# NinV/Background-Debiased-Video-CIL

Hardware: AMD Instinct MI355X
Metric: clips/sec fwd+bwd TSM-R50 8x224^2 bs32/GPU (higher is better)
Workload: dtype f32; 1 GPU; TSM-ResNet50 fwd+bwd+SGD step, synthetic 32x8x3x224x224 clips per GPU, 101 classes, SimpleLinear+CrossEntropyLoss, dropout 0.5, random-init weights; fp32 tensors, accumulators and results; conv products: fp32 via 3xbf16 split, 6 MFMA products, fp32 accumulate (dropped terms <= 2^-24 relative); conv_arith=bf16x3, clips_per_gpu=32, global_batch=32, parallelism=dp1

## Files before the change

### background-debiased-video-cil_amd/_lib.py

```python
from __future__ import annotations

import ctypes
import os
from ctypes import POINTER, Structure, c_char, c_char_p, c_float, c_int, c_int32, c_int64, c_size_t, c_uint16, c_uint64, c_void_p

_HERE = os.path.dirname(os.path.abspath(__file__))
_OVERRIDE = os.environ.get('BDVCIL_LIB_PATH')
LIB_PATH = _OVERRIDE or os.path.join(_HERE, 'csrc', 'libbdvcil_hip.so')
ABI_VERSION = 33

_lib = None


class ConvGeom(Structure):
    _fields_ = [(n, c_int32) for n in
                ('N', 'H', 'W', 'Cin', 'Ho', 'Wo', 'Cout', 'R', 'S', 'stride', 'pad', 'T', 'fold', 'pad_w', 'Rt', 'st_t', 'act_dtype')]

    def key(self):
        return tuple(getattr(self, n) for n, _ in self._fields_)


class ConvPlan(Structure):
    _fields_ = [(n, c_int32) for n in ('family', 'reads_planes', 'stat_rows', 'splits', 'pre_ok')] + [('kernel', c_char * 128)]


P = c_void_p
_F3 = c_float * 3


class ConvAffine(Structure):
    _fields_ = [('scale', c_void_p), ('shift', c_void_p), ('residual', c_void_p), ('relu', c_int32)]


class BnStatFuse(Structure):
    _fields_ = [('y', c_void_p), ('relu_mask', c_void_p), ('mean', c_void_p), ('invstd', c_void_p), ('partial', c_void_p),
                ('relu_scale', c_void_p), ('relu_shift', c_void_p)]

class JpegInfo(Structure):
    _fields_ = [('width', c_int32), ('height', c_int32), ('ncomp', c_int32), ('h', c_int32 * 3), ('v', c_int32 * 3),
                ('blocks_w', c_int32 * 3), ('blocks_h', c_int32 * 3), ('down_w', c_int32 * 3), ('down_h', c_int32 * 3),
                ('qt', (c_uint16 * 64) * 3), ('coef_offset', c_int64 * 3), ('coef_count', c_int64)]

    def geometry_key(self):
        return (self.width, self.height, self.ncomp, tuple(self.h), tuple(self.v))


SIGNATURES = {
    'bdv_last_error': (c_char_p, []),
    'bdv_abi_version': (c_int, []),
    'bdv_source_hash': (c_char_p, []),
    'bdv_conv_workspace_bytes': (c_size_t, [POINTER(ConvGeom), c_int]),
    'bdv_conv_plan_query': (c_int, [POINTER(ConvGeom), c_int, c_int, c_int, POINTER(ConvPlan)]),
    'bdv_conv_fprop': (c_int, [P, P, P, POINTER(ConvGeom), P, POINTER(ConvAffine), P, c_size_t, P]),
    'bdv_conv_dgrad': (c_int, [P, P, P, P, P, POINTER(ConvGeom), POINTER(BnStatFuse), P, c_size_t, P]),
    'bdv_conv_weight_planes_bytes': (c_size_t, [POINTER(ConvGeom)]),
    'bdv_conv_split_weights': (c_int, [P, POINTER(ConvGeom), P, P, P]),
    'bdv_conv_debug_force_tile': (c_int, [c_int]),
    'bdv_conv_fprop_pl': (c_int, [P, P, P, P, POINTER(ConvGeom), P, POINTER(ConvAffine), P, c_size_t, c_int, P, P, P]),
    'bdv_conv_dgrad_pl': (c_int, [P, P, P, P, P, P, POINTER(ConvGeom), POINTER(BnStatFuse), P, c_size_t, c_int, P]),
    'bdv_conv_wgrad': (c_int, [P, P, P, c_float, POINTER(ConvGeom), P, c_size_t, P]),
    'bdv_conv_wgrad_partial': (c_int, [P, P, POINTER(ConvGeom), P, c_size_t, P]),
    'bdv_conv_wgrad_partial_pl': (c_int, [P, P, POINTER(ConvGeom), P, c_size_t, c_int, P, P, P]),
    'bdv_wgrad_reduce_batched': (c_int, [P, P, P, P, c_int, c_float, P]),
    'bdv_f16x2_amax': (c_int, [P, c_int64, P, P]),
    'bdv_f16x2_scale': (c_float, [c_float]),
    'bdv_conv_split_weights_f16x2': (c_int, [P, POINTER(ConvGeom), P, P, P]),
    'bdv_conv_fprop_f16x2': (c_int, [P, P, P, P, P, POINTER(ConvGeom), P, POINTER(ConvAffine), P, c_size_t, P, P, P]),
    'bdv_conv_dgrad_f16x2': (c_int, [P, P, P, P, P, P, P, POINTER(ConvGeom), POINTER(BnStatFuse), P, c_size_t, P]),
    'bdv_conv_wgrad_partial_f16x2': (c_int, [P, P, P, P, POINTER(ConvGeom), P, c_size_t, P, P, P]),
    'bdv_bn_workspace_bytes': (c_size_t, [c_int64, c_int]),
    'bdv_bn_train_stats': (c_int, [P, c_int64, c_int, P, P, c_float, c_float, P, P, P, P, P, P, P, c_size_t, P]),
    'bdv_bn_train_finalize': (c_int, [P, c_int, c_int64, c_int, P, P, c_float, c_float, P, P, P, P, P, P, P]),
    'bdv_bn_eval_params': (c_int, [c_int, P, P, P, P, c_float, P, P, P]),
    'bdv_bn_apply': (c_int, [P, P, P, P, P, P, P, P, c_int64, c_int, c_int, c_int, P]),
    'bdv_bn_backward': (c_int, [P, P, P, P, P, P, P, P, P, c_float, c_int64, c_int, c_int, P, c_int, P, P, P, c_size_t, c_int, P]),
    'bdv_bn_finalize_scratch_bytes': (c_size_t, [c_int]),
    'bdv_bn_finalize_splits': (c_int, [c_int, c_int]),
    'bdv_bn_train_finalize_split': (c_int, [P, c_int, c_int64, c_int, P, P, c_float, c_float, P, P, P, P, P, P, c_int, P, c_size_t, P]),
    'bdv_bn_backward_split': (c_int, [P, P, P, P, P, P, P, P, P, c_float, c_int64, c_int, c_int, P, c_int, P, P, P, c_size_t, c_int,
                                      c_int, P, c_size_t, P]),
    'bdv_bn_pair_workspace_bytes': (c_size_t, [c_int64, c_int]),
    'bdv_bn_backward_pair': (c_int, [P, P, P, P, P, P, P, c_int, P, P, P, P, P, P, P, P, P, P, c_int64, c_int, P, c_size_t, c_int, c_int,
                                     P, c_size_t, P]),
    'bdv_bn_eval_backward': (c_int, [P, P, P, P, P, P, P, P, P, P, P, c_float, c_int64, c_int, P, c_size_t, c_int, c_int, P, c_size_t, P]),
    'bdv_bn_backward_maxpool_split': (c_int, [P, P, P, P, P, P, P, P, P, P, c_float, c_int, c_int, c_int, c_int, P, c_size_t, c_int,
                                              c_int, P, c_size_t, P]),
    'bdv_bn_backward_maxpool': (c_int, [P, P, P, P, P, P, P, P, P, P, c_float, c_int, c_int, c_int, c_int, P, c_size_t, c_int, P]),
    'bdv_relu_bwd': (c_int, [P, P, P, P, c_int64, c_int, P]),
    'bdv_add': (c_int, [P, P, P, c_int64, c_int, P]),
    'bdv_nchw3_to_nhwc4': (c_int, [P, P, c_int, c_int, c_int, P]),
# ... 37 lines not shown
    'bdv_lsc_loss': (c_int, [P, P, P, c_float, c_int, P, P, P, P, c_int, c_int, P]),
    'bdv_softce_loss': (c_int, [P, P, P, P, P, c_int, c_int, P]),
    'bdv_icarl_targets': (c_int, [P, P, c_int, P, P, c_int, c_int, P]),
    'bdv_acm_targets': (c_int, [P, P, P, c_float, P, c_int, c_int, P]),
    'bdv_softmax_mean': (c_int, [P, P, c_int, c_int, c_int, c_int, P]),
    'bdv_topk_acc': (c_int, [P, P, P, c_int, c_int, P]),
    'bdv_repr_from_features': (c_int, [P, P, P, c_int, c_int, c_int, c_int, P]),
    'bdv_nme_workspace_bytes': (c_size_t, [c_int, c_int]),
    'bdv_nme_classify': (c_int, [P, P, P, P, c_int, c_int, c_int, c_int, P, c_size_t, P]),
    'bdv_class_means': (c_int, [P, P, P, c_int, c_int, c_int, P]),
    'bdv_herding_workspace_bytes': (c_size_t, [c_int, c_int]),
    'bdv_herding_select': (c_int, [P, c_int, c_int, c_int, c_int, P, P, P, P, c_size_t, P]),
    'bdv_randaug_workspace_bytes': (c_size_t, [c_int, c_int, c_int, c_int]),
    'bdv_randaug_apply': (c_int, [P, P, P, P, c_int, c_int, c_int, c_int, P, c_size_t, P]),
    'bdv_reduce_workspace_bytes': (c_size_t, []),
    'bdv_kd_mse_fwd': (c_int, [P, P, P, c_int64, P, c_size_t, c_int, P]),
    'bdv_kd_mse_bwd': (c_int, [P, P, P, c_float, P, c_int64, c_int, P]),
    'bdv_multi_sqnorm': (c_int, [P, P, c_int, P, P, c_size_t, P]),
    'bdv_clip_coef': (c_int, [P, c_float, c_float, P, P]),
    'bdv_multi_sgd': (c_int, [P, P, P, P, P, P, c_int, c_float, c_float, P, P]),
    'bdv_gradcam_map': (c_int, [P, P, P, c_int, c_int, c_int, P]),
    'bdv_gradcam_minmax': (c_int, [P, c_int, c_int, c_int, c_int, c_int, c_int, P, P]),
    'bdv_gradcam_workspace_bytes': (c_size_t, [c_int, c_int, c_int]),
    'bdv_gradcam_render': (c_int, [P, P, c_int, c_int, c_int, c_int, c_int, c_int, P, P, P, c_float, _F3, _F3, P, P, P, P, P, c_int, P, P,
                                   c_size_t, P]),
}


class HipExtensionError(RuntimeError):
    pass


HASHED_SOURCES = ('conv_mfma.hip', 'bn.hip', 'pool_frontend.hip', 'head_loss.hip', 'repr.hip', 'augment.hip', 'optim.hip', 'jpeg.hip',
                  'background.hip', 'actor_cut_mix.hip', 'sim_cam.hip', 'ragged.hip', 'gradcam.hip', 'api_common.cpp', 'common.h', 'resize_linear.h', 'Makefile', '../../include/bdvcil_hip.h')


def source_hash():
    import hashlib
    h = hashlib.sha256()
    base = os.path.join(_HERE, 'csrc')
    for name in HASHED_SOURCES:
        path = os.path.join(base, name)
        if not os.path.exists(path):
            return None
        with open(path, 'rb') as f:
            h.update(f.read())
    return h.hexdigest()


def lib():
    global _lib
    if _lib is None:
        if not os.path.exists(LIB_PATH):
            raise HipExtensionError(
                f'HIP extension not built: {LIB_PATH} is missing. Run `python -c "import __graft_entry__ as g; '
                f'g.build()"` (or `make -C {os.path.dirname(LIB_PATH)}`). There is no CPU fallback.')
        handle = ctypes.CDLL(LIB_PATH)
        for name, (res, args) in SIGNATURES.items():
            fn = getattr(handle, name)
            fn.restype = res
            fn.argtypes = args
        if handle.bdv_abi_version() != ABI_VERSION:
            raise HipExtensionError(f'ABI mismatch: library {handle.bdv_abi_version()} != binding {ABI_VERSION}')
        want, have = source_hash(), handle.bdv_source_hash().decode()
        if want is not None and want != have and not _OVERRIDE:
            raise HipExtensionError(f'stale library: {LIB_PATH} was built from other sources (hash {have[:12]}, in-tree '
                                    f'{want[:12]}). Rebuild: make -C {os.path.dirname(LIB_PATH)}')
# ... 9 lines not shown
```

### background-debiased-video-cil_amd/csrc/conv_mfma.hip

```cpp
#include <stdlib.h>
#include <string.h>
#include "common.h"

#ifdef BDV_STAMPS
__device__ unsigned long long* g_stamp_buf = nullptr;
__device__ int g_stamp_cap = 0;
#define BDV_STAMP(slot)                                                                                                          \
  do {                                                                                                                           \
    if (threadIdx.x == 0 && g_stamp_buf != nullptr && (int)(blockIdx.x + gridDim.x * blockIdx.y) < g_stamp_cap) {                 \
      unsigned long long* q_ = g_stamp_buf + (size_t)(blockIdx.x + gridDim.x * blockIdx.y) * 8;                                  \
      if ((slot) == 4) asm volatile("s_waitcnt vmcnt(0)" ::: "memory");                                                          \
      q_[slot] = __builtin_amdgcn_s_memtime();                                                                                   \
      if ((slot) == 0) { q_[5] = __builtin_amdgcn_s_memrealtime(); q_[7] = __builtin_amdgcn_s_getreg((4 << 0) | (0 << 6) | (31 << 11)); } \
      if ((slot) == 4) q_[6] = __builtin_amdgcn_s_memrealtime();                                                                 \
    }                                                                                                                            \
  } while (0)
#else
#define BDV_STAMP(slot) do { } while (0)
#endif

namespace {

constexpr int BK = 32;

struct Geom {
  int N, H, W, Cin, Ho, Wo, Cout, R, S, stride, pad, pad_w, T, fold;
  int Rt, st_t;
  float rcp_RS, rcp_S;
  int M;
  int Ktot;
  float rcp_HoWo, rcp_Wo;
  int stagger;
};

typedef unsigned int u32x4 __attribute__((ext_vector_type(4)));
constexpr int kOOB = (int)0x80000000;

__device__ __forceinline__ float4 buf_load16(__amdgpu_buffer_rsrc_t rsrc, int voff, int soff) {
  const u32x4 v = __builtin_amdgcn_raw_buffer_load_b128(rsrc, voff, soff, 0);
  return make_float4(__uint_as_float(v.x), __uint_as_float(v.y), __uint_as_float(v.z), __uint_as_float(v.w));
}

__device__ __forceinline__ void buf_store16(__amdgpu_buffer_rsrc_t rsrc, int voff, float4 v) {
  u32x4 d;
  d.x = __float_as_uint(v.x);
  d.y = __float_as_uint(v.y);
  d.z = __float_as_uint(v.z);
  d.w = __float_as_uint(v.w);
  __builtin_amdgcn_raw_buffer_store_b128(d, rsrc, voff, 0, 0);
}

typedef unsigned int u32x2v __attribute__((ext_vector_type(2)));
template <int ES>
__device__ __forceinline__ float4 buf_ld4(__amdgpu_buffer_rsrc_t rsrc, int voff) {
  if constexpr (ES == 4) {
    return buf_load16(rsrc, voff, 0);
  } else {
    const u32x2v v = __builtin_amdgcn_raw_buffer_load_b64(rsrc, voff, 0, 0);
    return bdv_widen_bf16x4(v.x, v.y);
  }
}
template <int ES>
__device__ __forceinline__ void buf_st4(__amdgpu_buffer_rsrc_t rsrc, int voff, float4 v) {
  if constexpr (ES == 4) {
    buf_store16(rsrc, voff, v);
// ... 1663 lines not shown
      __syncthreads();
      store(0, PlSet0{});
      load(PlSet0{});
      mma(1);
      __syncthreads();
    }
  } else {
    for (; i + 4 < n; i += 2) {
      mma(0);
      store(1, PlSet1{});
      load(PlSet1{});
      __syncthreads();
      mma(1);
      store(0, PlSet0{});
      load(PlSet0{});
      __syncthreads();
    }
  }
  for (; i < n; i += 2) {
    mma(0);
    if (i + 1 < n) store(1, PlSet1{});
    if (i + 3 < n) load(PlSet1{});
    __syncthreads();
    if (i + 1 >= n) break;
    mma(1);
    if (i + 2 < n) store(0, PlSet0{});
    if (i + 4 < n) load(PlSet0{});
    __syncthreads();
  }
}

constexpr int pl_waves_per_simd(int waves, int np, bool fits128) { return np == 1 && waves == 8 && fits128 ? 4 : waves == 4 ? 2 : waves / 4; }

template <int BM, int BN, int WM, int WN, int NBUF, int NP = 3, bool PRE = false, int ES = 4, typename PT = Bf16Pieces>
__global__ __launch_bounds__(64 * WM * WN, pl_waves_per_simd(WM * WN, NP, BN == 64 || (BM == 128 && BN == 256))) void conv_fprop_pl_kernel(const void* __restrict__ x,
                                                                                      const unsigned short* __restrict__ wp,
                                                                                      void* __restrict__ y, Geom g, int NT, Work wk,
                                                                                      float* __restrict__ slab, FpropEpi epi,
                                                                                      PieceScales ps) {
  static_assert(!kF16<PT> || (NP == 2 && !PRE && ES == 4), "fp16 pieces: two per operand, fp32 tensors, no BatchNorm in the loader");
  constexpr int NTHR = 64 * WM * WN;
  constexpr int TM = BM / WM / 32, TN = BN / WN / 32;
  constexpr int KG = ES == 2 ? 4 : 8;
  constexpr int AP = BM * KG / NTHR;
  constexpr int BPP = (BN * 4 + NTHR - 1) / NTHR;
  constexpr int PA = BM * 64, PB = BN * 64, STAGE = NP * (PA + PB);
  constexpr int SMEM = NBUF * STAGE >= WM * 32 * BN * 4 ? NBUF * STAGE : WM * 32 * BN * 4;
  static_assert(AP >= 1 && SMEM <= 160 * 1024, "tile / epilogue staging do not fit");
  __shared__ __attribute__((aligned(16))) unsigned char smem_b[SMEM];
  float* const smem = reinterpret_cast<float*>(smem_b);

  BDV_STAMP(0);
  const int nk = g.Ktot / BK;
  const WorkItem it = get_work(blockIdx.x, wk, nk);
  const int mt = it.tile / NT, nt = it.tile - mt * NT;

  const int tid = threadIdx.x;
  const int lane = tid & 63, wave = tid >> 6;
  const int wm = wave / WN, wn = wave % WN;
  const int arow = tid / KG, kg = tid % KG;
  const int brow = tid >> 2, bc = tid & 3;
  const int HoWo = g.Ho * g.Wo;
  static_assert(ES == 4 || (NP == 1 && !PRE), "bf16 storage: single-product arithmetic only");
  const int frame_bytes = g.H * g.W * g.Cin * ES;
  const int plane_bytes = g.Cout * g.Ktot * 2;

  const __amdgpu_buffer_rsrc_t xr = __builtin_amdgcn_make_buffer_rsrc((void*)x, 0, g.N * frame_bytes, 0x00020000);
  const __amdgpu_buffer_rsrc_t wr = __builtin_amdgcn_make_buffer_rsrc((void*)wp, 0, 3 * plane_bytes, 0x00020000);

  int a_base[AP], a_t[AP], a_hi0[AP], a_wi0[AP];
#pragma unroll
  for (int p = 0; p < AP; ++p) {
    const int m = mt * BM + arow + (NTHR / KG) * p;
    const bool ok = m < g.M;
    int n, rem, ho, wo;
    fast_divmod(ok ? m : 0, HoWo, g.rcp_HoWo, n, rem);
    fast_divmod(rem, g.Wo, g.rcp_Wo, ho, wo);
    a_t[p] = n % g.T;
    a_hi0[p] = ok ? ho * g.stride - g.pad : -(1 << 20);
    a_wi0[p] = wo * g.stride - g.pad_w;
// ... 48 lines not shown
    chunk += wr_;
  };
  const int st_a = ES == 2 ? pl_off(arow, kg) : pl_off(arow, kg >> 1) + 8 * (kg & 1), st_b = pl_off(brow, bc);
  const int fa[2] = {pl_frag_off(32 * wm, 0, lane), pl_frag_off(32 * wm, 1, lane)};
  const int fb[2] = {pl_frag_off(32 * wn, 0, lane), pl_frag_off(32 * wn, 1, lane)};
  const float sc_a = f16x2_scale<PT>(ps.a);
  auto store = [&](int stage, auto set) __attribute__((always_inline)) {
    constexpr int SET = decltype(set)::value;
    unsigned char* const As = smem_b + stage * STAGE;
    unsigned char* const Bs = As + NP * PA;
#pragma unroll
    for (int p = 0; p < AP; ++p) {
      float4 v = ra[SET][p];
      if constexpr (PRE) {
        const bool ok = (pvalid[SET] >> p) & 1u;
        v.x = ok ? fmaxf(fmaf(v.x, psc[SET].x, psh[SET].x), 0.f) : 0.f;
        v.y = ok ? fmaxf(fmaf(v.y, psc[SET].y, psh[SET].y), 0.f) : 0.f;
        v.z = ok ? fmaxf(fmaf(v.z, psc[SET].z, psh[SET].z), 0.f) : 0.f;
        v.w = ok ? fmaxf(fmaf(v.w, psc[SET].w, psh[SET].w), 0.f) : 0.f;
      }
      if constexpr (ES == 2) *reinterpret_cast<float4*>(As + st_a + (NTHR / KG) * p * 64) = v;
      else pl_split_store_at<NP, PT>(As + st_a + (NTHR / KG) * p * 64, PA, v, sc_a);
    }
    if (b_active) {
#pragma unroll
      for (int pl = 0; pl < NP; ++pl)
#pragma unroll
        for (int q = 0; q < BPP; ++q) *reinterpret_cast<u32x4*>(Bs + st_b + (pl * PB + (NTHR / 4) * q * 64)) = rb[SET][pl * BPP + q];
    }
  };
  f32x16 acc[TM][TN];
  zero_acc<TM, TN>(acc);

  if constexpr (NBUF == 2) {
    pl_pipeline2(it.ke - it.kb, load, store, [&](int stage) __attribute__((always_inline)) {
      mma_stage_pl<BM, BN, WM, WN, NP, PT>(smem_b + stage * STAGE, smem_b + stage * STAGE + NP * PA, acc, fa, fb);
    }, g.stagger != 0 && wave >= WM * WN / 2);
  } else {
    load(PlSet0{});
    for (int kt = it.kb; kt < it.ke; ++kt) {
      __syncthreads();
      store(0, PlSet0{});
      __syncthreads();
      if (kt == it.kb) BDV_STAMP(1);
      if (kt + 1 < it.ke) load(PlSet0{});
      mma_stage_pl<BM, BN, WM, WN, NP, PT>(smem_b, smem_b + NP * PA, acc, fa, fb);
    }
  }
  BDV_STAMP(2);
  f16x2_unscale<PT>(acc, ps);

  if (it.pslot >= 0) {
    store_partial<TM, TN, NTHR>(slab, it.pslot, acc, tid);
    return;
  }
  fprop_epilogue<BM, BN, WM, WN, ES>(acc, smem, y, g, epi, mt, nt, tid);
  BDV_STAMP(3);
  BDV_STAMP(4);
}

template <int BM, int BN, int WM, int WN, int NBUF, int NP = 3, int ES = 4, typename PT = Bf16Pieces>
__global__ __launch_bounds__(64 * WM * WN, BM == 64 ? 4 : pl_waves_per_simd(WM * WN, NP, BN == 64)) void conv_dgrad_pl_kernel(const void* __restrict__ dy,
                                                                                      const unsigned short* __restrict__ dp,
                                                                                      void* __restrict__ dx,
                                                                                      const void* __restrict__ add_src,
                                                                                      const uint32_t* __restrict__ add_mask, Geom g,
                                                                                      int NT, Work wk, float* __restrict__ slab,
                                                                                      BnStat stat, PieceScales ps) {
  static_assert(!kF16<PT> || (NP == 2 && ES == 4), "fp16 pieces: two per operand, fp32 tensors");
  constexpr int NTHR = 64 * WM * WN;
  constexpr int TM = BM / WM / 32, TN = BN / WN / 32;
  constexpr int KG = ES == 2 ? 4 : 8;
  constexpr int AP = BM * KG / NTHR;
  constexpr int BPP = (BN * 4 + NTHR - 1) / NTHR;
  constexpr int PA = BM * 64, PB = BN * 64, STAGE = NP * (PA + PB);
  constexpr int SMEM = NBUF * STAGE >= WM * 32 * BN * 4 ? NBUF * STAGE : WM * 32 * BN * 4;
  static_assert(AP >= 1 && SMEM <= 160 * 1024, "tile / epilogue staging do not fit");
  __shared__ __attribute__((aligned(16))) unsigned char smem_b[SMEM];
  float* const smem = reinterpret_cast<float*>(smem_b);

  BDV_STAMP(0);
  const int st = g.stride;
  const int ph = blockIdx.y / st, pw = blockIdx.y - ph * st;
  const int Hc = (g.H - ph + st - 1) / st, Wc = (g.W - pw + st - 1) / st;
  const int Mc = g.N * Hc * Wc;
  const int MT = (Mc + BM - 1) / BM;
  const int r0 = (ph + g.pad) % st, s0 = (pw + g.pad_w) % st;
  const int nr = r0 < g.R ? (g.R - r0 + st - 1) / st : 0;
  const int ns = s0 < g.S ? (g.S - s0 + st - 1) / st : 0;
  const int bh = (ph + g.pad - r0) / st, bw = (pw + g.pad_w - s0) / st;
  const int ntap = nr * ns;
  const int nk = ntap * g.Cout / BK;

  int mt, nt;
  WorkItem it;
  if (st == 1) {
    it = get_work(blockIdx.x, wk, nk);
    mt = it.tile / NT;
    nt = it.tile - mt * NT;
  } else {
    const int id = blockIdx.x;
    const int xcd = id & 7, jj = id >> 3;
    mt = (jj / NT) * 8 + xcd;
    nt = jj % NT;
    if (mt >= MT) return;
    it.tile = 0;
    it.kb = 0;
    it.ke = nk;
    it.pslot = -1;
// ... 55 lines not shown
      for (int q = 0; q < BPP; ++q) rb[SET][pl * BPP + q] = __builtin_amdgcn_raw_buffer_load_b128(wr, b_base[q] + pl * plane_bytes, koff_b, 0);
    is += 1;
    const int w1 = (is == ns) ? 1 : 0;
    is = w1 ? 0 : is;
    ir += w1;
    const int w2 = (ir == nr) ? 1 : 0;
    ir = w2 ? 0 : ir;
    chunk += w2;
  };
  const int st_a = ES == 2 ? pl_off(arow, kg) : pl_off(arow, kg >> 1) + 8 * (kg & 1), st_b = pl_off(brow, bc);
  const int fa[2] = {pl_frag_off(32 * wm, 0, lane), pl_frag_off(32 * wm, 1, lane)};
  const int fb[2] = {pl_frag_off(32 * wn, 0, lane), pl_frag_off(32 * wn, 1, lane)};
  const float sc_a = f16x2_scale<PT>(ps.a);
  auto store = [&](int stage, auto set) __attribute__((always_inline)) {
    constexpr int SET = decltype(set)::value;
    unsigned char* const As = smem_b + stage * STAGE;
    unsigned char* const Bs = As + NP * PA;
#pragma unroll
    for (int p = 0; p < AP; ++p) {
      if constexpr (ES == 2) *reinterpret_cast<float4*>(As + st_a + (NTHR / KG) * p * 64) = ra[SET][p];
      else pl_split_store_at<NP, PT>(As + st_a + (NTHR / KG) * p * 64, PA, ra[SET][p], sc_a);
    }
    if (b_active) {
#pragma unroll
      for (int pl = 0; pl < NP; ++pl)
#pragma unroll
        for (int q = 0; q < BPP; ++q) *reinterpret_cast<u32x4*>(Bs + st_b + (pl * PB + (NTHR / 4) * q * 64)) = rb[SET][pl * BPP + q];
    }
  };

  f32x16 acc[TM][TN];
  zero_acc<TM, TN>(acc);

  if (it.ke > it.kb) {
    if constexpr (NBUF == 2) {
      pl_pipeline2(it.ke - it.kb, load, store, [&](int stage) __attribute__((always_inline)) {
        mma_stage_pl<BM, BN, WM, WN, NP, PT>(smem_b + stage * STAGE, smem_b + stage * STAGE + NP * PA, acc, fa, fb);
      }, g.stagger != 0 && wave >= WM * WN / 2);
    } else {
      load(PlSet0{});
      for (int kt = it.kb; kt < it.ke; ++kt) {
        __syncthreads();
        store(0, PlSet0{});
        __syncthreads();
        if (kt == it.kb) BDV_STAMP(1);
        if (kt + 1 < it.ke) load(PlSet0{});
        mma_stage_pl<BM, BN, WM, WN, NP, PT>(smem_b, smem_b + NP * PA, acc, fa, fb);
      }
    }
  }
  BDV_STAMP(2);
  f16x2_unscale<PT>(acc, ps);
  if (it.pslot >= 0) {
    store_partial<TM, TN, NTHR>(slab, it.pslot, acc, tid);
    return;
  }
  constexpr bool EPI_PIPE = TM * TN <= 4 && NP >= 2 && BM != 64;
  dgrad_epilogue<BM, BN, WM, WN, true, ES, EPI_PIPE>(acc, smem, tid, dx, add_src, add_mask, g, mt, nt, Mc, stat, [&](int mrow) {
    if (st == 1) return mrow;
    const int n = mrow / HcWc;
    const int rem = mrow - n * HcWc;
    const int hc = rem / Wc;
    return (n * g.H + hc * st + ph) * g.W + (rem - hc * Wc) * st + pw;
  });
  BDV_STAMP(3);
  BDV_STAMP(4);
}
// ... 269 lines not shown
  }
}


int check_geom(const bdv_conv_geom* g, const char* who) {
  BDV_REQUIRE(g != nullptr, "%s: geom is NULL", who);
  BDV_REQUIRE(g->N > 0 && g->H > 0 && g->W > 0 && g->Ho > 0 && g->Wo > 0, "%s: non-positive extent", who);
  BDV_REQUIRE(g->Cin > 0 && g->Cin % 4 == 0, "%s: Cin=%d must be a positive multiple of 4", who, g->Cin);
  BDV_REQUIRE(g->Cout > 0 && g->Cout % 64 == 0, "%s: Cout=%d must be a multiple of 64", who, g->Cout);
  BDV_REQUIRE(g->R > 0 && g->S > 0 && g->pad >= 0, "%s: bad filter", who);
  BDV_REQUIRE(g->stride == 1 || g->stride == 2, "%s: stride %d unsupported", who, g->stride);
  const int pad_w = g->pad_w < 0 ? g->pad : g->pad_w;
  BDV_REQUIRE(g->Ho == (g->H + 2 * g->pad - g->R) / g->stride + 1 && g->Wo == (g->W + 2 * pad_w - g->S) / g->stride + 1,
              "%s: Ho/Wo inconsistent with H/W/pad/stride", who);
  BDV_REQUIRE(g->Cin % BK == 0 || g->Cin == 4, "%s: Cin=%d must be a multiple of 32 (or exactly 4)", who, g->Cin);
  if (g->Rt > 1) {
    BDV_REQUIRE(g->Cin == 4 && g->fold == 0, "%s: temporal taps (Rt=%d) are implemented for the stem only (Cin = 4, no shift)", who, g->Rt);
    BDV_REQUIRE((g->st_t == 1 || g->st_t == 2) && g->T > 0 && g->N % g->T == 0, "%s: Rt=%d needs st_t 1|2 and N %% T == 0 (T = output frames per clip)", who, g->Rt);
    BDV_REQUIRE((int64_t)g->N * g->st_t * g->H * g->W * g->Cin < (1ll << 29), "%s: input exceeds 2^29 elements", who);
  }
  if (g->fold > 0) {
    BDV_REQUIRE(g->fold % 4 == 0 && 2 * g->fold <= g->Cin, "%s: fold=%d must be a multiple of 4 and <= Cin/2", who,
                g->fold);
    BDV_REQUIRE(g->T > 0 && g->N % g->T == 0, "%s: N=%d not a multiple of T=%d", who, g->N, g->T);
    BDV_REQUIRE(g->Cin % BK == 0, "%s: temporal shift needs Cin %% 32 == 0", who);
  }
  BDV_REQUIRE((int64_t)g->N * g->H * g->W * g->Cin < (1ll << 29) && (int64_t)g->N * g->Ho * g->Wo * g->Cout < (1ll << 29),
              "%s: tensor exceeds 2^29 elements", who);
  BDV_REQUIRE((int64_t)g->Cout * g->R * g->S * g->Cin < (1ll << 29), "%s: weight tensor too large", who);
  BDV_REQUIRE((int64_t)g->N * g->Ho * g->Wo < (1ll << 22) || g->Cin == 4, "%s: more than 2^22 output pixels", who);
  return BDV_OK;
}

static bool pl_stagger_enabled() {
  const char* e = getenv("BDVCIL_STAGGER");
  return e == nullptr || atoi(e) != 0;
}

Geom make_geom(const bdv_conv_geom* g) {
  Geom d;
  d.stagger = pl_stagger_enabled() ? 1 : 0;
  d.N = g->N; d.H = g->H; d.W = g->W; d.Cin = g->Cin; d.Ho = g->Ho; d.Wo = g->Wo; d.Cout = g->Cout;
  d.R = g->R; d.S = g->S; d.stride = g->stride; d.pad = g->pad; d.pad_w = g->pad_w < 0 ? g->pad : g->pad_w;
  d.T = (g->fold > 0 || g->Rt > 1) ? g->T : 1;
  d.fold = g->fold;
  d.Rt = g->Rt > 1 ? g->Rt : 1;
  d.st_t = g->Rt > 1 ? g->st_t : 1;
  d.rcp_RS = 1.0f / (float)(g->R * g->S);
  d.rcp_S = 1.0f / (float)g->S;
  d.M = 0; d.Ktot = 0;
  d.rcp_HoWo = 1.0f / (float)(g->Ho * g->Wo);
  d.rcp_Wo = 1.0f / (float)g->Wo;
  return d;
}

bool debug_plan() {
  static const bool on = getenv("BDVCIL_DEBUG_PLAN") != nullptr;
  return on;
}

Work plan_work(int tiles, int nk, double iter_us, size_t seg_bytes, size_t ws_bytes, int per_cu = 3) {
  const int cus = 256, W = per_cu * cus;
  Work wk;
  const int q = tiles / W, r = tiles - q * W;
  wk.dp_tiles = tiles;
  wk.rem_tiles = 0;
  wk.split = 1;
  if (r == 0 || nk < 4) return wk;
  auto tail_time = [&](int blocks, double iters) {
    const int full = blocks / W, rest = blocks - full * W;
    const int c = (rest + cus - 1) / cus;
    const double e = c >= 3 ? 1.0 : (c == 2 ? 0.92 : 0.6);
    return iters * iter_us * (3.0 * full + (c > 0 ? c / e : 0.0));
  };
// ... 613 lines not shown
    if (p.wide)
      hipLaunchKernelGGL((conv_dgrad_fixup_kernel<128, 128, 2, 2>), fg, dim3(256), 0, s, (const float*)slab, dx, add_src, add_mask_src, g, p.NT, p.wk, stat);
    else
      hipLaunchKernelGGL((conv_dgrad_fixup_kernel<128, 64, 2, 2>), fg, dim3(256), 0, s, (const float*)slab, dx, add_src, add_mask_src, g, p.NT, p.wk, stat);
    BDV_LAUNCH_CHECK("bdv_conv_dgrad(fixup)");
  }
  return BDV_OK;
}
}

extern "C" int bdv_conv_dgrad(const float* dy, const float* w, float* dx, const float* add_src,
                              const uint32_t* add_mask_src, const bdv_conv_geom* gg, const bdv_bn_stat_fuse* bn_stat,
                              void* workspace, size_t workspace_bytes, void* stream) {
  return conv_dgrad_impl(dy, w, dx, add_src, add_mask_src, gg, bn_stat, workspace, workspace_bytes, stream, 0);
}

extern "C" size_t bdv_conv_weight_planes_bytes(const bdv_conv_geom* gg) {
  if (check_geom(gg, "bdv_conv_weight_planes_bytes")) return 0;
  return (size_t)3 * gg->Cout * gg->R * gg->S * gg->Cin * sizeof(unsigned short);
}

#ifdef BDV_STAMPS
extern "C" int bdv_debug_set_stamps(void* buf, int cap_workgroups) {
  unsigned long long* p = (unsigned long long*)buf;
  if (hipMemcpyToSymbol(HIP_SYMBOL(g_stamp_buf), &p, sizeof(p)) != hipSuccess) return -1;
  if (hipMemcpyToSymbol(HIP_SYMBOL(g_stamp_cap), &cap_workgroups, sizeof(int)) != hipSuccess) return -1;
  return 0;
}
#endif

extern "C" int bdv_conv_debug_force_tile(int cfg) {
  BDV_REQUIRE(cfg >= -1 && cfg <= kNumPlCfg, "bdv_conv_debug_force_tile: cfg %d (-1 automatic, 0 = 128x256, 1 = 256x128, 2 = 256x256, 3 = 256x64, 4 = 64x128 (dgrad), 5 = 128x128 (four waves), 6 = none)", cfg);
  g_pl_tile_forced = cfg;
  return BDV_OK;
}

extern "C" int bdv_conv_split_weights(const float* w, const bdv_conv_geom* gg, void* planes_fprop, void* planes_dgrad, void* stream) {
  if (int e = check_geom(gg, "bdv_conv_split_weights")) return e;
  BDV_REQUIRE(w && (planes_fprop || planes_dgrad), "bdv_conv_split_weights: null pointer");
  BDV_REQUIRE(gg->Cin % 32 == 0 && gg->Cout % 32 == 0, "bdv_conv_split_weights: Cin=%d and Cout=%d must be multiples of 32", gg->Cin, gg->Cout);
  BDV_REQUIRE(bdv_aligned16(w) && bdv_aligned16(planes_fprop) && bdv_aligned16(planes_dgrad), "bdv_conv_split_weights: alignment");
  const dim3 grid(gg->Cin / 32, gg->Cout / 32, gg->R * gg->S);
  hipLaunchKernelGGL(split_weights_kernel, grid, dim3(256), 0, (hipStream_t)stream, w, (unsigned short*)planes_fprop,
                     (unsigned short*)planes_dgrad, gg->Cout, gg->R * gg->S, gg->Cin);
  BDV_LAUNCH_CHECK("bdv_conv_split_weights");
  return BDV_OK;
}

namespace {
const unsigned* f16x2_weight_amax(const void* planes, const bdv_conv_geom* gg) {
  return (const unsigned*)((const unsigned char*)planes + (size_t)2 * gg->Cout * gg->R * gg->S * gg->Cin * sizeof(unsigned short));
}

int conv_fprop_pl_impl(const void* x, const float* w, const void* planes_fprop, void* y, const bdv_conv_geom* gg, float* bn_partial,
                       const bdv_conv_affine* affine, void* workspace, size_t workspace_bytes, int pieces, const float* pre_scale,
                       const float* pre_shift, const unsigned* amax_x, void* stream) {
  const bool pre = pre_scale != nullptr;
  const ConvPlan cp = plan_conv(gg, kFprop, pieces, pre);
  if (cp.family < 0) return BDV_EINVAL;
  if (pieces == kArithF16x2 && !cp.f16) pieces = 3;
  const PieceScales ps = {cp.f16 ? amax_x : nullptr, cp.f16 ? f16x2_weight_amax(planes_fprop, gg) : nullptr};
  BDV_REQUIRE(!cp.f16 || (amax_x != nullptr && planes_fprop != nullptr), "bdv_conv_fprop_f16x2: null pointer (amax_x, planes_fprop)");
  const bool h16 = gg->act_dtype == BDV_ACT_BF16;
  if (pre) {
    BDV_REQUIRE(pre_shift != nullptr && cp.pre_ok,
                "bdv_conv_fprop_pl: a producer BatchNorm in the loader needs the plane kernels (pieces 3, no temporal shift, Cin %% 32 == 0)");
// ... 401 lines not shown
```

### include/bdvcil_hip.h

```cpp
#ifndef BDVCIL_HIP_H
#define BDVCIL_HIP_H

#include <stddef.h>
#include <stdint.h>

#ifdef __cplusplus
extern "C" {
#endif

#define BDV_OK 0
#define BDV_EINVAL (-1)
#define BDV_EWORKSPACE (-2)

#define BDV_ACT_F32 0
#define BDV_ACT_BF16 1

typedef struct bdv_conv_geom {
  int32_t N;
  int32_t H, W;
  int32_t Cin;
  int32_t Ho, Wo;
  int32_t Cout;
  int32_t R, S;
  int32_t stride;
// ... 25 lines not shown
  int32_t stat_rows;
  int32_t splits;
  int32_t pre_ok;
  char kernel[128];
} bdv_conv_plan;
int bdv_conv_plan_query(const bdv_conv_geom* g, int kind, int arith, int pre, bdv_conv_plan* out);

typedef struct bdv_conv_affine {
  const float* scale;
  const float* shift;
  const void* residual;
  int32_t relu;
} bdv_conv_affine;
int bdv_conv_fprop(const float* x, const float* w, float* y, const bdv_conv_geom* g, float* bn_partial,
                   const bdv_conv_affine* affine, void* workspace, size_t workspace_bytes, void* stream);

typedef struct bdv_bn_stat_fuse {
  const void* y;
  const uint32_t* relu_mask;
  const float* mean;
  const float* invstd;
  float* partial;
  const float* relu_scale;
  const float* relu_shift;
} bdv_bn_stat_fuse;

int bdv_conv_dgrad(const float* dy, const float* w, float* dx, const float* add_src,
                   const uint32_t* add_mask_src, const bdv_conv_geom* g, const bdv_bn_stat_fuse* bn_stat, void* workspace,
                   size_t workspace_bytes, void* stream);

size_t bdv_conv_weight_planes_bytes(const bdv_conv_geom* g);
int bdv_conv_split_weights(const float* w, const bdv_conv_geom* g, void* planes_fprop, void* planes_dgrad, void* stream);
int bdv_conv_debug_force_tile(int cfg);
int bdv_conv_fprop_pl(const void* x, const float* w, const void* planes_fprop, void* y, const bdv_conv_geom* g,
                      float* bn_partial, const bdv_conv_affine* affine, void* workspace, size_t workspace_bytes, int pieces,
                      const float* pre_scale, const float* pre_shift, void* stream);
int bdv_conv_dgrad_pl(const void* dy, const float* w, const void* planes_dgrad, void* dx, const void* add_src,
                      const uint32_t* add_mask_src, const bdv_conv_geom* g, const bdv_bn_stat_fuse* bn_stat, void* workspace,
                      size_t workspace_bytes, int pieces, void* stream);

#define BDV_ARITH_F16X2 4
int bdv_f16x2_amax(const float* t, int64_t n, void* amax, void* stream);
float bdv_f16x2_scale(float amax);
int bdv_conv_split_weights_f16x2(const float* w, const bdv_conv_geom* g, void* planes_fprop, void* planes_dgrad, void* stream);
int bdv_conv_fprop_f16x2(const void* x, const void* amax_x, const float* w, const void* planes_fprop, void* y,
                         const bdv_conv_geom* g, float* bn_partial, const bdv_conv_affine* affine, void* workspace,
                         size_t workspace_bytes, const float* pre_scale, const float* pre_shift, void* stream);
int bdv_conv_dgrad_f16x2(const void* dy, const void* amax_dy, const float* w, const void* planes_dgrad, void* dx,
                         const void* add_src, const uint32_t* add_mask_src, const bdv_conv_geom* g,
                         const bdv_bn_stat_fuse* bn_stat, void* workspace, size_t workspace_bytes, void* stream);
int bdv_conv_wgrad_partial_f16x2(const void* dy, const void* amax_dy, const void* x, const void* amax_x, const bdv_conv_geom* g,
                                 void* slab, size_t slab_bytes, const float* pre_scale, const float* pre_shift, void* stream);

int bdv_conv_wgrad(const float* dy, const float* x, float* dw, float beta, const bdv_conv_geom* g, void* workspace,
                   size_t workspace_bytes, void* stream);
#define BDV_MAX_REDUCE_ITEMS 32
int bdv_conv_wgrad_partial(const float* dy, const float* x, const bdv_conv_geom* g, void* slab, size_t slab_bytes,
                           void* stream);
int bdv_wgrad_reduce_batched(const float* const* slabs, float* const* dws, const int* splits, const int64_t* numels, int n,
                             float beta, void* stream);
int bdv_conv_wgrad_partial_pl(const void* dy, const void* x, const bdv_conv_geom* g, void* slab, size_t slab_bytes,
                              int pieces, const float* pre_scale, const float* pre_shift, void* stream);

size_t bdv_bn_workspace_bytes(int64_t M, int C);
int bdv_bn_train_stats(const float* y, int64_t M, int C, const float* gamma, const float* beta,
                       float eps, float momentum, float* running_mean, float* running_var,
// ... 181 lines not shown
```

Before: 617.4 clips/s.

## Reuse one staged activation row-run across the three horizontal filter taps in 3x3 convs

For the 256x64 planar tile on stride-1 3x3 convolutions, fprop and dgrad now load and split one contiguous activation run of BM+2 rows per filter row into LDS. The three horizontal taps then read it through shifted offsets, with zeroed separator rows at image-width boundaries, instead of reloading and resplitting the activations for every tap. Weights are staged separately and a new pipeline interleaves the three parts. This targets cutting global activation loads and bf16 split work per tap, at the cost of more LDS per block, more complex index setup and a narrower set of tiles it applies to. A debug switch turns it off, and it is on by default.

```diff
diff --git a/background-debiased-video-cil_amd/_lib.py b/background-debiased-video-cil_amd/_lib.py
--- a/background-debiased-video-cil_amd/_lib.py
+++ b/background-debiased-video-cil_amd/_lib.py
@@ -56,6 +56,7 @@
     'bdv_conv_weight_planes_bytes': (c_size_t, [POINTER(ConvGeom)]),
     'bdv_conv_split_weights': (c_int, [P, POINTER(ConvGeom), P, P, P]),
     'bdv_conv_debug_force_tile': (c_int, [c_int]),
+    'bdv_conv_debug_row_run': (c_int, [c_int]),
     'bdv_conv_fprop_pl': (c_int, [P, P, P, P, POINTER(ConvGeom), P, POINTER(ConvAffine), P, c_size_t, c_int, P, P, P]),
     'bdv_conv_dgrad_pl': (c_int, [P, P, P, P, P, P, POINTER(ConvGeom), POINTER(BnStatFuse), P, c_size_t, c_int, P]),
     'bdv_conv_wgrad': (c_int, [P, P, P, c_float, POINTER(ConvGeom), P, c_size_t, P]),
@@ -159,7 +160,7 @@
 
 
 HASHED_SOURCES = ('conv_mfma.hip', 'bn.hip', 'pool_frontend.hip', 'head_loss.hip', 'repr.hip', 'augment.hip', 'optim.hip', 'jpeg.hip',
-                  'background.hip', 'actor_cut_mix.hip', 'sim_cam.hip', 'ragged.hip', 'gradcam.hip', 'api_common.cpp', 'common.h', 'resize_linear.h', 'Makefile', '../../include/bdvcil_hip.h')
+                  'background.hip', 'actor_cut_mix.hip', 'sim_cam.hip', 'ragged.hip', 'gradcam.hip', 'api_common.cpp', 'common.h', 'resize_linear.h', 'conv_row_run.h', 'Makefile', '../../include/bdvcil_hip.h')
 
 
 def source_hash():
diff --git a/background-debiased-video-cil_amd/csrc/conv_mfma.hip b/background-debiased-video-cil_amd/csrc/conv_mfma.hip
--- a/background-debiased-video-cil_amd/csrc/conv_mfma.hip
+++ b/background-debiased-video-cil_amd/csrc/conv_mfma.hip
@@ -1,6 +1,7 @@
 #include <stdlib.h>
 #include <string.h>
 #include "common.h"
+#include "conv_row_run.h"
 
 #ifdef BDV_STAMPS
 __device__ unsigned long long* g_stamp_buf = nullptr;
@@ -31,6 +32,7 @@
   int Ktot;
   float rcp_HoWo, rcp_Wo;
   int stagger;
+  int row_run;
 };
 
 typedef unsigned int u32x4 __attribute__((ext_vector_type(4)));
@@ -1760,6 +1762,168 @@
 
 constexpr int pl_waves_per_simd(int waves, int np, bool fits128) { return np == 1 && waves == 8 && fits128 ? 4 : waves == 4 ? 2 : waves / 4; }
 
+constexpr int kRrRows = 256 + 96;
+constexpr int kRrDataRows = kRrRows - 1;
+template <int BM, int BN, int NP, int ES, bool PRE>
+constexpr bool kRowRunTile = BM == 256 && BN == 64 && NP >= 2 && ES == 4 && !PRE;
+template <int BM, int BN, int NP>
+constexpr int kRowRunSmem = 2 * NP * (kRrRows * 64 + BN * 64);
+static_assert(kRowRunSmem<256, 64, 3> <= 160 * 1024, "row-run images + weight stages of the 256x64 tile do not fit the LDS");
+static_assert(rowrun::fits(256, 3, kRrDataRows) && !rowrun::fits(256, 2, kRrDataRows), "row-run fallback bound: W >= 3 takes the path");
+
+template <int BM, int BN, int WM, int WN, int NP, typename PT, int PAR>
+__device__ __forceinline__ void mma_stage_rr(const unsigned char* __restrict__ As, const unsigned char* __restrict__ Bs,
+                                             f32x16 (&acc)[BM / WM / 32][BN / WN / 32], const int (&fa)[BM / WM / 32][2],
+                                             const int (&fb)[2]) {
+  constexpr int TM = BM / WM / 32, TN = BN / WN / 32;
+  constexpr int PB = BN * 64;
+#pragma unroll
+  for (int s = 0; s < BK / 16; ++s) {
+    bf16x8_t a[NP][TM], b[NP][TN];
+#pragma unroll
+    for (int p = 0; p < NP; ++p) {
+#pragma unroll
+      for (int i = 0; i < TM; ++i) a[p][i] = *reinterpret_cast<const bf16x8_t*>(As + fa[i][s] + p * PAR);
+#pragma unroll
+      for (int j = 0; j < TN; ++j) b[p][j] = *reinterpret_cast<const bf16x8_t*>(Bs + fb[s] + (p * PB + 32 * WN * j * 64));
+    }
+#pragma unroll
+    for (int i = 0; i < TM; ++i)
+#pragma unroll
+      for (int j = 0; j < TN; ++j) {
+        if constexpr (NP == 3) {
+          acc[i][j] = __builtin_amdgcn_mfma_f32_32x32x16_bf16(a[1][i], b[1][j], acc[i][j], 0, 0, 0);
+          acc[i][j] = __builtin_amdgcn_mfma_f32_32x32x16_bf16(a[0][i], b[2][j], acc[i][j], 0, 0, 0);
+          acc[i][j] = __builtin_amdgcn_mfma_f32_32x32x16_bf16(a[2][i], b[0][j], acc[i][j], 0, 0, 0);
+        }
+        if constexpr (NP >= 2) {
+          acc[i][j] = mfma_piece<PT>(a[0][i], b[1][j], acc[i][j]);
+          acc[i][j] = mfma_piece<PT>(a[1][i], b[0][j], acc[i][j]);
+        }
+        acc[i][j] = mfma_piece<PT>(a[0][i], b[0][j], acc[i][j]);
+      }
+  }
+}
+
+using RrPart0 = std::integral_constant<int, 0>;
+using RrPart1 = std::integral_constant<int, 1>;
+using RrPart2 = std::integral_constant<int, 2>;
+template <typename LoadA, typename NextA, typename StoreA, typename LoadB, typename StoreB, typename MmaF>
+__device__ __forceinline__ void pl_pipeline_rr(int n, int s0, LoadA&& loadA, NextA&& nextA, StoreA&& storeA, LoadB&& loadB,
+                                               StoreB&& storeB, MmaF&& mma, bool late) {
+  loadA(RrPart0{});
+  loadA(RrPart1{});
+  loadA(RrPart2{});
+  nextA();
+  loadB(PlSet0{});
+  storeA(0, RrPart0{});
+  storeA(0, RrPart1{});
+  storeA(0, RrPart2{});
+  loadA(RrPart0{});
+  loadA(RrPart1{});
+  loadA(RrPart2{});
+  nextA();
+  storeB(0, PlSet0{});
+  loadB(PlSet1{});
+  loadB(PlSet0{});
+  if (s0 >= 1) {
+    storeA(1, RrPart0{});
+    loadA(RrPart0{});
+  }
+  if (s0 >= 2) {
+    storeA(1, RrPart1{});
+    loadA(RrPart1{});
+  }
+  __syncthreads();
+  BDV_STAMP(1);
+  auto step = [&](auto set, auto part, auto is_late, int img) __attribute__((always_inline)) {
+    constexpr int SET = decltype(set)::value, S = decltype(part)::value;
+    using Other = std::integral_constant<int, SET ^ 1>;
+    if constexpr (decltype(is_late)::value) {
+      storeB(SET ^ 1, Other{});
+      loadB(Other{});
+      storeA(img ^ 1, part);
+      loadA(part);
+      mma(img, part, SET);
+    } else {
+      mma(img, part, SET);
+      storeB(SET ^ 1, Other{});
+      loadB(Other{});
+      storeA(img ^ 1, part);
+      loadA(part);
+    }
+    if constexpr (S == 2) nextA();
+    __syncthreads();
+  };
+  int i = 0, abuf = 0, s = s0;
+  auto any_step = [&]() __attribute__((always_inline)) {
+    auto by_order = [&](auto set, auto part) __attribute__((always_inline)) {
+      if (late) step(set, part, std::true_type{}, abuf);
+      else step(set, part, std::false_type{}, abuf);
+    };
+    switch ((i & 1) * 3 + s) {
+      case 0: by_order(PlSet0{}, RrPart0{}); break;
+      case 1: by_order(PlSet0{}, RrPart1{}); break;
+      case 2: by_order(PlSet0{}, RrPart2{}); break;
+      case 3: by_order(PlSet1{}, RrPart0{}); break;
+      case 4: by_order(PlSet1{}, RrPart1{}); break;
+      default: by_order(PlSet1{}, RrPart2{}); break;
+    }
+    i += 1;
+    s += 1;
+    if (s == 3) {
+      s = 0;
+      abuf ^= 1;
+    }
+  };
+  auto rounds = [&](auto is_late) __attribute__((always_inline)) {
+    for (; i + 6 <= n; i += 6) {
+      step(PlSet0{}, RrPart0{}, is_late, abuf);
+      step(PlSet1{}, RrPart1{}, is_late, abuf);
+      step(PlSet0{}, RrPart2{}, is_late, abuf);
+      step(PlSet1{}, RrPart0{}, is_late, abuf ^ 1);
+      step(PlSet0{}, RrPart1{}, is_late, abuf ^ 1);
+      step(PlSet1{}, RrPart2{}, is_late, abuf ^ 1);
+    }
+  };
+  if (s0 == 0) {
+    if (late) rounds(std::true_type{});
+    else rounds(std::false_type{});
+  }
+  while (i < n) any_step();
+}
+
+template <int BM, int WM, int NP, int NTHR, int AP>
+__device__ __forceinline__ void rr_setup(unsigned char* __restrict__ smem_b, int m0, int W, float rcp_W, int tid, int wm,
+                                         int (&st)[AP], int (&fa)[3][BM / WM / 32][2]) {
+  constexpr int PAR = kRrRows * 64;
+  const int c0 = rowrun::col0(m0, W);
+  const int lane = tid & 63, arow = tid >> 3, kg = tid & 7;
+#pragma unroll
+  for (int p = 0; p < AP; ++p) {
+    const int j = arow + (NTHR / 8) * p;
+    int q, rm;
+    fast_divmod(c0 + j, W, rcp_W, q, rm);
+    st[p] = pl_off(j < BM + 2 ? j + q : kRrDataRows, kg >> 1) + 8 * (kg & 1);
+  }
+#pragma unroll
+  for (int i = 0; i < BM / WM / 32; ++i) {
+    const int j = 32 * WM * i + 32 * wm + (lane & 31) + 1;
+    int q, rm;
+    fast_divmod(c0 + j, W, rcp_W, q, rm);
+#pragma unroll
+    for (int d = 0; d < 3; ++d)
+#pragma unroll
+      for (int s = 0; s < 2; ++s) fa[d][i][s] = pl_off(j + q + d - 1, 2 * s + (lane >> 5));
+  }
+  const int nsep = rowrun::num_sep(BM, c0, W);
+  for (int idx = tid; idx < nsep * 2 * NP * 4; idx += NTHR) {
+    const int k = idx / (2 * NP * 4), rest = idx - k * (2 * NP * 4);
+    *reinterpret_cast<float4*>(smem_b + (rest >> 2) * PAR + rowrun::sep_row(k + 1, c0, W) * 64 + 16 * (rest & 3)) =
+        make_float4(0.f, 0.f, 0.f, 0.f);
+  }
+}
+
 template <int BM, int BN, int WM, int WN, int NBUF, int NP = 3, bool PRE = false, int ES = 4, typename PT = Bf16Pieces>
 __global__ __launch_bounds__(64 * WM * WN, pl_waves_per_simd(WM * WN, NP, BN == 64 || (BM == 128 && BN == 256))) void conv_fprop_pl_kernel(const void* __restrict__ x,
                                                                                       const unsigned short* __restrict__ wp,
@@ -1773,7 +1937,9 @@
   constexpr int AP = BM * KG / NTHR;
   constexpr int BPP = (BN * 4 + NTHR - 1) / NTHR;
   constexpr int PA = BM * 64, PB = BN * 64, STAGE = NP * (PA + PB);
-  constexpr int SMEM = NBUF * STAGE >= WM * 32 * BN * 4 ? NBUF * STAGE : WM * 32 * BN * 4;
+  constexpr int SMEM0 = NBUF * STAGE >= WM * 32 * BN * 4 ? NBUF * STAGE : WM * 32 * BN * 4;
+  constexpr bool RR = kRowRunTile<BM, BN, NP, ES, PRE> && NBUF == 2;
+  constexpr int SMEM = RR && kRowRunSmem<BM, BN, NP> > SMEM0 ? kRowRunSmem<BM, BN, NP> : SMEM0;
   static_assert(AP >= 1 && SMEM <= 160 * 1024, "tile / epilogue staging do not fit");
   __shared__ __attribute__((aligned(16))) unsigned char smem_b[SMEM];
   float* const smem = reinterpret_cast<float*>(smem_b);
@@ -1888,7 +2054,84 @@
   f32x16 acc[TM][TN];
   zero_acc<TM, TN>(acc);
 
-  if constexpr (NBUF == 2) {
+  bool rr_done = false;
+  if constexpr (RR) {
+    if (g.row_run != 0 && g.S == 3 && g.stride == 1 && g.pad_w == 1 && g.Rt == 1 && rowrun::fits(BM, g.W, kRrDataRows)) {
+      constexpr int PAR = kRrRows * 64;
+      constexpr int APR = (BM + 2 + 63) / 64;
+      static_assert(NTHR == 512 && KG == 8 && APR == 5, "row run: 64 run entries per pass, parts {0,1} {2,3} {4}");
+      unsigned char* const Bst = smem_b + 2 * NP * PAR;
+      int st_r[APR], fa3[3][TM][2];
+      rr_setup<BM, WM, NP, NTHR, APR>(smem_b, mt * BM, g.W, g.rcp_Wo, tid, wm, st_r, fa3);
+      int e_base[APR], e_t[APR], e_h[APR];
+#pragma unroll
+      for (int p = 0; p < APR; ++p) {
+        const int j = arow + 64 * p, m = mt * BM - 1 + j;
+        const bool ok = j < BM + 2 && m >= 0 && m < g.M;
+        int n, rem, ho, wo;
+        fast_divmod(ok ? m : 0, HoWo, g.rcp_HoWo, n, rem);
+        fast_divmod(rem, g.Wo, g.rcp_Wo, ho, wo);
+        e_t[p] = n % g.T;
+        e_h[p] = ok ? ho - g.pad : -(1 << 20);
+        e_base[p] = ((n * g.H + ho - g.pad) * g.W + wo) * g.Cin * ES + 16 * kg;
+      }
+      const int nchunk = g.Cin / BK;
+      float4 re[APR];
+      int chunk_a = it.kb / RS, r_a = (it.kb - chunk_a * RS) / 3;
+      auto loadA = [&](auto part) __attribute__((always_inline)) {
+        constexpr int P0 = 2 * decltype(part)::value, P1 = P0 == 4 ? APR : P0 + 2;
+        const int cls = shift_class(chunk_a * BK + 4 * kg, g.fold);
+        const int koff = (r_a * g.W * g.Cin + chunk_a * BK) * ES + cls * frame_bytes;
+        const bool live = chunk_a < nchunk;
+#pragma unroll
+        for (int p = P0; p < P1; ++p) {
+          const bool v = live && (unsigned)(e_h[p] + r_a) < (unsigned)g.H && (unsigned)(e_t[p] + cls) < (unsigned)g.T;
+          re[p] = buf_load16(xr, (e_base[p] + koff) | (v ? 0 : kOOB), 0);
+        }
+      };
+      auto nextA = [&]() __attribute__((always_inline)) {
+        r_a += 1;
+        const int w_ = (r_a == g.R) ? 1 : 0;
+        r_a = w_ ? 0 : r_a;
+        chunk_a += w_;
+      };
+      auto storeA = [&](int img, auto part) __attribute__((always_inline)) {
+        constexpr int P0 = 2 * decltype(part)::value, P1 = P0 == 4 ? APR : P0 + 2;
+        unsigned char* const As = smem_b + img * (NP * PAR);
+#pragma unroll
+        for (int p = P0; p < P1; ++p) {
+          pl_split_store_at<NP, PT>(As + st_r[p], PAR, re[p], sc_a);
+        }
+      };
+      auto loadB = [&](auto set) __attribute__((always_inline)) {
+        constexpr int SET = decltype(set)::value;
+        const int off = kt_w < it.ke ? 0 : kOOB;
+        const int koff_b = kt_w * g.Cout * 64;
+#pragma unroll
+        for (int pl = 0; pl < NP; ++pl)
+#pragma unroll
+          for (int q = 0; q < BPP; ++q)
+            rb[SET][pl * BPP + q] = __builtin_amdgcn_raw_buffer_load_b128(wr, (b_base[q] + pl * plane_bytes) | off, off ? 0 : koff_b, 0);
+        kt_w += 1;
+      };
+      auto storeB = [&](int stage, auto set) __attribute__((always_inline)) {
+        constexpr int SET = decltype(set)::value;
+        if (b_active) {
+#pragma unroll
+          for (int pl = 0; pl < NP; ++pl)
+#pragma unroll
+            for (int q = 0; q < BPP; ++q)
+              *reinterpret_cast<u32x4*>(Bst + stage * (NP * PB) + st_b + (pl * PB + (NTHR / 4) * q * 64)) = rb[SET][pl * BPP + q];
+        }
+      };
+      pl_pipeline_rr(it.ke - it.kb, s, loadA, nextA, storeA, loadB, storeB, [&](int img, auto part, int stage) __attribute__((always_inline)) {
+        mma_stage_rr<BM, BN, WM, WN, NP, PT, PAR>(smem_b + img * (NP * PAR), Bst + stage * (NP * PB), acc, fa3[decltype(part)::value], fb);
+      }, g.stagger != 0 && wave >= WM * WN / 2);
+      rr_done = true;
+    }
+  }
+  if (rr_done) {
+  } else if constexpr (NBUF == 2) {
     pl_pipeline2(it.ke - it.kb, load, store, [&](int stage) __attribute__((always_inline)) {
       mma_stage_pl<BM, BN, WM, WN, NP, PT>(smem_b + stage * STAGE, smem_b + stage * STAGE + NP * PA, acc, fa, fb);
     }, g.stagger != 0 && wave >= WM * WN / 2);
@@ -1930,7 +2173,9 @@
   constexpr int AP = BM * KG / NTHR;
   constexpr int BPP = (BN * 4 + NTHR - 1) / NTHR;
   constexpr int PA = BM * 64, PB = BN * 64, STAGE = NP * (PA + PB);
-  constexpr int SMEM = NBUF * STAGE >= WM * 32 * BN * 4 ? NBUF * STAGE : WM * 32 * BN * 4;
+  constexpr int SMEM0 = NBUF * STAGE >= WM * 32 * BN * 4 ? NBUF * STAGE : WM * 32 * BN * 4;
+  constexpr bool RR = kRowRunTile<BM, BN, NP, ES, false> && NBUF == 2;
+  constexpr int SMEM = RR && kRowRunSmem<BM, BN, NP> > SMEM0 ? kRowRunSmem<BM, BN, NP> : SMEM0;
   static_assert(AP >= 1 && SMEM <= 160 * 1024, "tile / epilogue staging do not fit");
   __shared__ __attribute__((aligned(16))) unsigned char smem_b[SMEM];
   float* const smem = reinterpret_cast<float*>(smem_b);
@@ -2052,7 +2297,90 @@
   f32x16 acc[TM][TN];
   zero_acc<TM, TN>(acc);
 
-  if (it.ke > it.kb) {
+  bool rr_done = false;
+  if constexpr (RR) {
+    if (g.row_run != 0 && st == 1 && g.S == 3 && g.pad_w == 1 && it.ke > it.kb && rowrun::fits(BM, g.W, kRrDataRows)) {
+      constexpr int PAR = kRrRows * 64;
+      constexpr int APR = (BM + 2 + 63) / 64;
+      static_assert(NTHR == 512 && KG == 8 && APR == 5, "row run: 64 run entries per pass, parts {0,1} {2,3} {4}");
+      unsigned char* const Bst = smem_b + 2 * NP * PAR;
+      int st_r[APR], fa3[3][TM][2];
+      rr_setup<BM, WM, NP, NTHR, APR>(smem_b, mt * BM, g.W, g.rcp_Wo, tid, wm, st_r, fa3);
+      int e_base[APR], e_h[APR];
+#pragma unroll
+      for (int p = 0; p < APR; ++p) {
+        const int j = arow + 64 * p, m = mt * BM - 1 + j;
+        const bool ok = j < BM + 2 && m >= 0 && m < Mc;
+        const int mm = ok ? m : 0;
+        const int n = mm / HcWc;
+        const int rem = mm - n * HcWc;
+        const int hc = rem / Wc, wc = rem - hc * Wc;
+        e_h[p] = ok ? hc + bh : -(1 << 20);
+        e_base[p] = ((n * g.Ho + hc + bh) * g.Wo + wc) * g.Cout * ES + 16 * kg;
+      }
+      float4 re[APR];
+      int chunk_a = it.kb / ntap, r_a = (it.kb - chunk_a * ntap) / 3;
+      int kt_b = it.kb;
+      auto loadA = [&](auto part) __attribute__((always_inline)) {
+        constexpr int P0 = 2 * decltype(part)::value, P1 = P0 == 4 ? APR : P0 + 2;
+        const int koff = (chunk_a * BK - r_a * g.Wo * g.Cout) * ES;
+        const bool live = chunk_a < nchunk;
+#pragma unroll
+        for (int p = P0; p < P1; ++p) {
+          const bool v = live && (unsigned)(e_h[p] - r_a) < (unsigned)g.Ho;
+          re[p] = buf_load16(yr, (e_base[p] + koff) | (v ? 0 : kOOB), 0);
+        }
+      };
+      auto nextA = [&]() __attribute__((always_inline)) {
+        r_a += 1;
+        const int w_ = (r_a == nr) ? 1 : 0;
+        r_a = w_ ? 0 : r_a;
+        chunk_a += w_;
+      };
+      auto storeA = [&](int img, auto part) __attribute__((always_inline)) {
+        constexpr int P0 = 2 * decltype(part)::value, P1 = P0 == 4 ? APR : P0 + 2;
+        unsigned char* const As = smem_b + img * (NP * PAR);
+#pragma unroll
+        for (int p = P0; p < P1; ++p) {
+          pl_split_store_at<NP, PT>(As + st_r[p], PAR, re[p], sc_a);
+        }
+      };
+      auto loadB = [&](auto set) __attribute__((always_inline)) {
+        constexpr int SET = decltype(set)::value;
+        const int off = kt_b < it.ke ? 0 : kOOB;
+        const int tap = (r0 + ir * st) * g.S + (s0 + is * st);
+        const int koff_b = (tap * nchunk + chunk) * g.Cin * 64;
+#pragma unroll
+        for (int pl = 0; pl < NP; ++pl)
+#pragma unroll
+          for (int q = 0; q < BPP; ++q)
+            rb[SET][pl * BPP + q] = __builtin_amdgcn_raw_buffer_load_b128(wr, (b_base[q] + pl * plane_bytes) | off, off ? 0 : koff_b, 0);
+        kt_b += 1;
+        is += 1;
+        const int w1 = (is == ns) ? 1 : 0;
+        is = w1 ? 0 : is;
+        ir += w1;
+        const int w2 = (ir == nr) ? 1 : 0;
+        ir = w2 ? 0 : ir;
+        chunk += w2;
+      };
+      auto storeB = [&](int stage, auto set) __attribute__((always_inline)) {
+        constexpr int SET = decltype(set)::value;
+        if (b_active) {
+#pragma unroll
+          for (int pl = 0; pl < NP; ++pl)
+#pragma unroll
+            for (int q = 0; q < BPP; ++q)
+              *reinterpret_cast<u32x4*>(Bst + stage * (NP * PB) + st_b + (pl * PB + (NTHR / 4) * q * 64)) = rb[SET][pl * BPP + q];
+        }
+      };
+      pl_pipeline_rr(it.ke - it.kb, is, loadA, nextA, storeA, loadB, storeB, [&](int img, auto part, int stage) __attribute__((always_inline)) {
+        mma_stage_rr<BM, BN, WM, WN, NP, PT, PAR>(smem_b + img * (NP * PAR), Bst + stage * (NP * PB), acc, fa3[2 - decltype(part)::value], fb);
+      }, g.stagger != 0 && wave >= WM * WN / 2);
+      rr_done = true;
+    }
+  }
+  if (it.ke > it.kb && !rr_done) {
     if constexpr (NBUF == 2) {
       pl_pipeline2(it.ke - it.kb, load, store, [&](int stage) __attribute__((always_inline)) {
         mma_stage_pl<BM, BN, WM, WN, NP, PT>(smem_b + stage * STAGE, smem_b + stage * STAGE + NP * PA, acc, fa, fb);
@@ -2388,6 +2716,7 @@
   return BDV_OK;
 }
 
+int g_pl_row_run = 1;
 static bool pl_stagger_enabled() {
   const char* e = getenv("BDVCIL_STAGGER");
   return e == nullptr || atoi(e) != 0;
@@ -2396,6 +2725,7 @@
 Geom make_geom(const bdv_conv_geom* g) {
   Geom d;
   d.stagger = pl_stagger_enabled() ? 1 : 0;
+  d.row_run = g_pl_row_run;
   d.N = g->N; d.H = g->H; d.W = g->W; d.Cin = g->Cin; d.Ho = g->Ho; d.Wo = g->Wo; d.Cout = g->Cout;
   d.R = g->R; d.S = g->S; d.stride = g->stride; d.pad = g->pad; d.pad_w = g->pad_w < 0 ? g->pad : g->pad_w;
   d.T = (g->fold > 0 || g->Rt > 1) ? g->T : 1;
@@ -3075,6 +3405,12 @@
 extern "C" int bdv_conv_debug_force_tile(int cfg) {
   BDV_REQUIRE(cfg >= -1 && cfg <= kNumPlCfg, "bdv_conv_debug_force_tile: cfg %d (-1 automatic, 0 = 128x256, 1 = 256x128, 2 = 256x256, 3 = 256x64, 4 = 64x128 (dgrad), 5 = 128x128 (four waves), 6 = none)", cfg);
   g_pl_tile_forced = cfg;
+  return BDV_OK;
+}
+
+extern "C" int bdv_conv_debug_row_run(int on) {
+  BDV_REQUIRE(on == 0 || on == 1, "bdv_conv_debug_row_run: on = %d (1 = one activation image per filter row, 0 = the per-tap loader)", on);
+  g_pl_row_run = on;
   return BDV_OK;
 }
 
diff --git a/background-debiased-video-cil_amd/csrc/conv_row_run.h b/background-debiased-video-cil_amd/csrc/conv_row_run.h
--- /dev/null
+++ b/background-debiased-video-cil_amd/csrc/conv_row_run.h
@@ -0,0 +1,18 @@
+#pragma once
+
+#if defined(__HIPCC__) || defined(__CUDACC__)
+#define BDV_RR_HD __host__ __device__
+#else
+#define BDV_RR_HD
+#endif
+
+namespace rowrun {
+
+BDV_RR_HD constexpr int col0(int m0, int W) { return (m0 + W - 1) % W; }
+BDV_RR_HD constexpr int lds_row(int j, int c0, int W) { return j + (c0 + j) / W; }
+BDV_RR_HD constexpr int num_sep(int bm, int c0, int W) { return (c0 + bm + 1) / W; }
+BDV_RR_HD constexpr int sep_row(int k, int c0, int W) { return k * (W + 1) - c0 - 1; }
+BDV_RR_HD constexpr int rows_bound(int bm, int W) { return bm + 3 + bm / W; }
+BDV_RR_HD constexpr bool fits(int bm, int W, int cap) { return rows_bound(bm, W) <= cap; }
+
+}
diff --git a/include/bdvcil_hip.h b/include/bdvcil_hip.h
--- a/include/bdvcil_hip.h
+++ b/include/bdvcil_hip.h
@@ -81,6 +81,7 @@
 size_t bdv_conv_weight_planes_bytes(const bdv_conv_geom* g);
 int bdv_conv_split_weights(const float* w, const bdv_conv_geom* g, void* planes_fprop, void* planes_dgrad, void* stream);
 int bdv_conv_debug_force_tile(int cfg);
+int bdv_conv_debug_row_run(int on);
 int bdv_conv_fprop_pl(const void* x, const float* w, const void* planes_fprop, void* y, const bdv_conv_geom* g,
                       float* bn_partial, const bdv_conv_affine* affine, void* workspace, size_t workspace_bytes, int pieces,
                       const float* pre_scale, const float* pre_shift, void* stream);
```

New measurement: 624.3 clips/s, median of 6. 1.1% higher.
